# pablojara/kubernetesNetAwareScheduler

Measured on AMD Instinct MI355X. Metric: pod-node pair scores/sec and placements/sec at 10k nodes x 100k pods, higher is better.
Workload: dtype i8xi8->i32; 1 GPU; C3: 10000 nodes x 100000 pods, dense i8 latency + traffic, racks of 32 / zones of 16 racks, 8 peers per pod, clusterloader2-shaped requests; nodes=10000, pods=100000, parallelism=node-sharded x1, candidates_per_pod=8

## Files before the change

kubernetesnetawarescheduler_amd/csrc/k_cost.hip:

```cpp
#include "klist.h"

#include <type_traits>

namespace nas {
namespace {

typedef int v4i __attribute__((ext_vector_type(4)));
typedef int v16i __attribute__((ext_vector_type(16)));
typedef float v16f __attribute__((ext_vector_type(16)));
typedef float v4f __attribute__((ext_vector_type(4)));
typedef __bf16 bf16x8 __attribute__((ext_vector_type(8)));

constexpr int BM = COST_BM;
constexpr int BN = COST_BN;
constexpr int BKB = COST_BKB;
constexpr int PG_NARROW = 4;
constexpr int PG_WIDE = 2;
constexpr int WIDE_PODS = 384;
template <int DT>
constexpr bool mfma16() { return DT == NAS_DT_BF16; }
template <int DT>
struct Mma;

template <>
struct Mma<NAS_DT_I8> {
    using acc_t = v16i;
    using acc4_t = v4i;
    static __device__ __forceinline__ acc_t mma(v4i a, v4i b, acc_t c) {
        return __builtin_amdgcn_mfma_i32_32x32x32_i8(a, b, c, 0, 0, 0);
    }
    static __device__ __forceinline__ acc4_t mma16(v4i a, v4i b, acc4_t c) {
        return __builtin_amdgcn_mfma_i32_16x16x64_i8(a, b, c, 0, 0, 0);
    }
    static __device__ __forceinline__ unsigned okey(int x) { return (unsigned)x ^ 0x80000000u; }
};

template <>
struct Mma<NAS_DT_BF16> {
    using acc_t = v16f;
    using acc4_t = v4f;
    static __device__ __forceinline__ acc_t mma(v4i a, v4i b, acc_t c) {
        return __builtin_amdgcn_mfma_f32_32x32x16_bf16(__builtin_bit_cast(bf16x8, a),
                                                        __builtin_bit_cast(bf16x8, b), c, 0, 0, 0);
    }
    static __device__ __forceinline__ acc4_t mma16(v4i a, v4i b, acc4_t c) {
        return __builtin_amdgcn_mfma_f32_16x16x32_bf16(__builtin_bit_cast(bf16x8, a),
                                                        __builtin_bit_cast(bf16x8, b), c, 0, 0, 0);
    }
    static __device__ __forceinline__ unsigned okey(float x) {
        x = x + 0.0f;
        const unsigned u = __float_as_uint(x);
        return (u & 0x80000000u) ? ~u : (u | 0x80000000u);
    }
};

__device__ __forceinline__ void glds16(const void *g, void *l) {
    __builtin_amdgcn_global_load_lds((const void __attribute__((address_space(1))) *)g,
                                     (void __attribute__((address_space(3))) *)l, 16, 0, 0);
}

__device__ __forceinline__ unsigned lds_off(const void *p) {
    return (unsigned)(uintptr_t)(const __attribute__((address_space(3))) void *)p;
}
__device__ __forceinline__ void glds16_s(const void *sbase, unsigned voff, unsigned ldsa) {
    unsigned keep;
    asm volatile("s_mov_b32 %0, m0\n\ts_mov_b32 m0, %3\n\ts_nop 0\n\t"
                 "global_load_lds_dwordx4 %1, %2\n\ts_mov_b32 m0, %0"
                 : "=&s"(keep)
                 : "v"(voff), "s"(sbase), "s"(ldsa)
                 : "memory");
}

__device__ __forceinline__ unsigned umed3(unsigned a, unsigned b, unsigned c) {
    unsigned d;
    asm("v_med3_u32 %0, %1, %2, %3" : "=v"(d) : "v"(a), "v"(b), "v"(c));
    return d;
}

template <int DT, bool RMAP, int NWN, bool FUSE>
__global__ void __launch_bounds__(128 * NWN, 1)
k_cost_topk(const unsigned char *__restrict__ Lt, const unsigned char *__restrict__ WA, int Kb,
            int n_mt, int n_nt, int p0, int Pp, const u64 *__restrict__ mask,
            u64 *__restrict__ partial, u64 *__restrict__ pbound, int node_base,
            const int *__restrict__ dyn_start, int dyn_hi, const int *__restrict__ dyn_hi_ptr,
            Ovf ov, const int *__restrict__ rowmap, FitSrc fs, unsigned *__restrict__ cc) {
    static_assert(NWN == 4 || NWN == 6, "the 8- and 12-wave layouts");
    constexpr int NW = 2 * NWN;
    constexpr int NI = 2;
    constexpr int WPODS = 32 * NI;
    constexpr int BNK = NWN * WPODS;
    constexpr bool WIDE = BNK > BN;
    static_assert(!WIDE || (!RMAP && FUSE), "the wide tile serves the main pass only");
    static_assert(!FUSE || !RMAP, "the fused fit: main-range launches");
    constexpr int STG = (BM + BNK) * BKB;
    constexpr int PG = WIDE ? PG_WIDE : PG_NARROW;
    constexpr int PPWA = (BM / 8 + NW - 1) / NW;
    constexpr int PPWB = (BNK / 8 + NW - 1) / NW;
    constexpr int PPW = PPWB;
    using M = Mma<DT>;
    using acc_t = typename M::acc_t;
    constexpr bool M16 = mfma16<DT>();
    constexpr int AM = M16 ? 8 : 4;
    constexpr int AN = M16 ? 2 * NI : NI;
    constexpr int AR = M16 ? 4 : 16;
    constexpr int PB = M16 ? 16 : 32;
    using accb_t = std::conditional_t<M16, typename M::acc4_t, acc_t>;
    extern __shared__ __attribute__((aligned(16))) unsigned char lds[];
    constexpr int FIT_LDS_OFF = 32768;
    static_assert(FIT_LDS_OFF >= NWN * NI * 32 * 9 * 8 &&
                  FIT_LDS_OFF + NW * AN * 2 * 64 * 8 <= 2 * STG, "fused-fit LDS words");

    const int nwg = n_mt * n_nt;
    const int b = blockIdx.x;
    const int xcd = b & 7, q8 = nwg >> 3, r8 = nwg & 7;
    const int v = (xcd < r8 ? xcd * (q8 + 1) : r8 * (q8 + 1) + (xcd - r8) * q8) + (b >> 3);
    const int gsize = PG * n_mt;
    const int g = v / gsize, r = v % gsize;
    const int first_nt = g * PG;
    const int pg = min(n_nt - first_nt, PG);
    const int mt = r / pg;
    const int nt = first_nt + r % pg;
    const int cb = blockIdx.y;
    if constexpr (FUSE) {
        fs.cap += (size_t)cb * 3 * fs.N;
        fs.req += (size_t)cb * 3 * Pp;
    }
    Lt += (size_t)cb * n_mt * BM * Kb;
    WA += (size_t)cb * Pp * Kb;
    mask += (size_t)cb * (n_mt * BM / 64) * Pp;
    partial += (size_t)cb * n_mt * Pp * KC;
    pbound += (size_t)cb * n_mt * Pp;
    if (dyn_start) {
        const int s = dyn_start[cb * STATUS_INTS];
        if (s < 0) return;
        if (dyn_hi_ptr) dyn_hi = dyn_hi_ptr[cb * STATUS_INTS];
        p0 = s / BN * BN;
        if (p0 + nt * BNK >= dyn_hi) return;
    }
    const int p_end = (BNK != BN && !dyn_start) ? dyn_hi : 0x7fffffff;

    const int tid = threadIdx.x;
    int lane = tid & 63;
    const int w = WIDE ? __builtin_amdgcn_readfirstlane(tid >> 6) : tid >> 6;
    const int wm = w / NWN, wn = w % NWN;

    const unsigned char *Ag = Lt + (size_t)mt * BM * Kb;
    const unsigned char *Bg = WA + (size_t)(p0 + nt * BNK) * Kb;

    const int srow_in = lane >> 3;
    const int sq = lane & 7;
    auto abuf = [&](int b) -> unsigned char * { return lds + b * STG; };
    auto bbuf = [&](int b) -> unsigned char * { return lds + b * STG + BM * BKB; };
    const unsigned loffn = (unsigned)(srow_in * Kb) +
                           ((unsigned)(sq ^ ((4 * (w & 1) + (srow_in >> 1)) & 7)) << 4);
    auto pieceA = [&](int buf, int k0, int j) {
        if (BM / 8 % NW && j * NW + w >= BM / 8) return;
        const int r0 = (j * NW + w) * 8;
        const int ru = __builtin_amdgcn_readfirstlane(r0);
        glds16_s(Ag + (size_t)ru * Kb + k0, loffn,
                 __builtin_amdgcn_readfirstlane(lds_off(abuf(buf) + r0 * BKB)));
    };
    int bpod[PPW];
    if constexpr (RMAP) {
#pragma unroll
        for (int j = 0; j < PPW; ++j)
            bpod[j] = rowmap[min(p0 + nt * BNK + (j * NW + w) * 8 + srow_in, dyn_hi - 1)];
    }
    auto pieceB = [&](int buf, int k0, int j) {
        if (BNK / 8 % NW && j * NW + w >= BNK / 8) return;
        const int r0 = (j * NW + w) * 8;
        if constexpr (!RMAP) {
            const int ru = __builtin_amdgcn_readfirstlane(r0);
            glds16_s(Bg + (size_t)ru * Kb + k0, loffn,
                     __builtin_amdgcn_readfirstlane(lds_off(bbuf(buf) + r0 * BKB)));
            return;
        }
        const int row = r0 + srow_in;
        const int c = sq ^ ((row >> 1) & 7);
        const unsigned char *src = RMAP ? WA + (size_t)bpod[j] * Kb : Bg + (size_t)row * Kb;
        glds16(src + k0 + c * 16, bbuf(buf) + r0 * BKB);
    };
    const int wu = __builtin_amdgcn_readfirstlane(w);
    const unsigned loff = (unsigned)(srow_in * Kb) +
                          ((unsigned)(sq ^ ((4 * (wu & 1) + (srow_in >> 1)) & 7)) << 4);
    auto piece6 = [&](int buf, int k0, int j) {
        const int pj = j * NW + wu;
        if (pj >= (BM + BNK) / 8) return;
        const unsigned char *base = pj < BM / 8 ? Ag + (size_t)pj * 8 * Kb
                                                : Bg + (size_t)(pj - BM / 8) * 8 * Kb;
        glds16_s(base + k0, loff, __builtin_amdgcn_readfirstlane(lds_off(lds + buf * STG + pj * 8 * BKB)));
    };
    auto stageA = [&](int buf, int k0) {
        if constexpr (WIDE) {
#pragma unroll
            for (int j = 0; j < ((BM + BNK) / 8 + NW - 1) / NW; ++j) piece6(buf, k0, j);
        } else {
#pragma unroll
            for (int j = 0; j < PPWA; ++j) pieceA(buf, k0, j);
        }
    };
    auto stageB = [&](int buf, int k0) {
        if constexpr (!WIDE) {
#pragma unroll
            for (int j = 0; j < PPW; ++j) pieceB(buf, k0, j);
        }
    };

    int rq[FUSE ? AN : 1][3];
    int fcap[2][3];
    auto fit_issue = [&]() {
#pragma unroll
        for (int ni = 0; ni < AN; ++ni) {
            const int pod = min(p0 + nt * BNK + wn * WPODS + ni * PB + (lane & (PB - 1)), p_end - 1);
#pragma unroll
            for (int r = 0; r < 3; ++r) rq[ni][r] = fs.req[(size_t)r * Pp + pod];
        }
#pragma unroll
        for (int mi2 = 0; mi2 < 2; ++mi2) {
            const int nl = mt * BM + wm * 128 + mi2 * 64 + lane;
#pragma unroll
            for (int r = 0; r < 3; ++r)
                fcap[mi2][r] = nl < fs.nloc ? __hip_atomic_load(const_cast<int *>(fs.cap) + (size_t)r * fs.N + fs.n0 + nl,
                                                                __ATOMIC_RELAXED, __HIP_MEMORY_SCOPE_AGENT)
                                            : -1;
        }
    };
    auto fit_slot = [&](int ni, int mi2) -> u64 * {
        return reinterpret_cast<u64 *>(lds + FIT_LDS_OFF) + ((w * AN + ni) * 2 + mi2) * 64 + lane;
    };
    auto fit_words = [&]() {
#pragma unroll
        for (int mi2 = 0; mi2 < 2; ++mi2) {
            const bool real = mt * BM + wm * 128 + mi2 * 64 + lane < fs.nloc;
            const u64 valid = __builtin_amdgcn_ballot_w64(real);
            int mn[3], mx[3];
#pragma unroll
            for (int r = 0; r < 3; ++r) {
                int a = real ? fcap[mi2][r] : 0x7fffffff, x = real ? fcap[mi2][r] : (int)0x80000000;
#pragma unroll
                for (int o = 32; o; o >>= 1) {
                    a = min(a, __shfl_xor(a, o));
                    x = max(x, __shfl_xor(x, o));
                }
                mn[r] = __builtin_amdgcn_readfirstlane(a);
                mx[r] = __builtin_amdgcn_readfirstlane(x);
            }
#pragma unroll
            for (int ni = 0; ni < AN; ++ni) {
                const int a = rq[ni][0], bq = rq[ni][1], d = rq[ni][2];
                const bool all = a <= mn[0] && bq <= mn[1] && d <= mn[2];
                const bool none = a > mx[0] || bq > mx[1] || d > mx[2];
                u64 word = all ? valid : 0ull;
                u64 rest = __builtin_amdgcn_ballot_w64(!all && !none) & ((1ull << PB) - 1);
                while (rest) {
                    const int i = (int)__builtin_ctzll(rest);
                    rest &= rest - 1;
                    const int ra = __builtin_amdgcn_readlane(a, i), rb = __builtin_amdgcn_readlane(bq, i);
                    const int rd = __builtin_amdgcn_readlane(d, i);
                    const u64 m = __builtin_amdgcn_ballot_w64(ra <= fcap[mi2][0]) &
                                  __builtin_amdgcn_ballot_w64(rb <= fcap[mi2][1]) &
                                  __builtin_amdgcn_ballot_w64(rd <= fcap[mi2][2]);
                    if ((lane & (PB - 1)) == i) word = m;
                }
                *fit_slot(ni, mi2) = word;
            }
        }
    };

    u64 mwp[AN][2];
    auto load_mask = [&]() __attribute__((always_inline)) {
        if constexpr (!FUSE) {
#pragma unroll
            for (int ni = 0; ni < AN; ++ni)
#pragma unroll
                for (int mi2 = 0; mi2 < 2; ++mi2) {
                    const int pod = min(p0 + nt * BNK + wn * WPODS + ni * PB + (lane & (PB - 1)), p_end - 1);
                    const int chunk = (mt * BM + wm * 128 + mi2 * 64) >> 6;
                    mwp[ni][mi2] = mask[(size_t)chunk * Pp + pod];
                }
        }
    };
    accb_t acc[AM][AN];
#pragma unroll
    for (int i = 0; i < AM; ++i)
#pragma unroll
        for (int j = 0; j < AN; ++j) acc[i][j] = accb_t{};
    int fr = lane & (PB - 1), fh = lane / PB;
    constexpr bool OVF_ROUND2 = WIDE || !FUSE;
    if constexpr (OVF_ROUND2 && DT == NAS_DT_I8) {
        if (ov.ptr) {
            const int cnt_lim = ov.row_count ? *ov.row_count : 0x7fffffff;
            const signed char *lr = ov.Lr + (size_t)cb * ov.N * (n_mt * BM) + mt * BM + wm * 128 + 4 * fh;
#pragma unroll
            for (int ni = 0; ni < AN; ++ni) {
                const int r = p0 + nt * BNK + wn * WPODS + ni * PB + fr;
                int beg = 0, end = 0;
                if (r < cnt_lim && r < p_end) {
                    const int pod = (ov.row_pod ? ov.row_pod[r] : r) + cb * Pp;
                    beg = ov.ptr[pod];
                    end = ov.ptr[pod + 1];
                }
#pragma unroll
                for (int mi = 0; mi < AM; ++mi)
                    for (int j = beg; j < end; ++j) {
                        const int e = ov.e[j];
                        const signed char *row = lr + (size_t)ov.m[j] * (n_mt * BM) + mi * (128 / AM);
#pragma unroll
                        for (int g = 0; g < AR / 4; ++g) {
                            const int v = *reinterpret_cast<const int *>(row + 8 * g);
#pragma unroll
                            for (int c = 0; c < 4; ++c)
                                acc[mi][ni][4 * g + c] += e * (int)(signed char)(v >> (8 * c));
                        }
                    }
            }
        }
    }
    auto seed_ovf = [&]() __attribute__((always_inline)) {
        if constexpr (!OVF_ROUND2 && DT == NAS_DT_I8) {
            if (ov.ptr) {
                const int cnt_lim = ov.row_count ? *ov.row_count : 0x7fffffff;
                const signed char *lr = ov.Lr + (size_t)cb * ov.N * (n_mt * BM) + mt * BM + wm * 128 + 4 * fh;
                auto bounds = [&](int ni, int &beg, int &end) {
                    const int r = p0 + nt * BNK + wn * WPODS + ni * PB + fr;
                    beg = end = 0;
                    if (r < cnt_lim && r < p_end) {
                        const int pod = (ov.row_pod ? ov.row_pod[r] : r) + cb * Pp;
                        beg = ov.ptr[pod];
                        end = ov.ptr[pod + 1];
                    }
                };
                {
                    int beg[AN], end[AN];
#pragma unroll
                    for (int ni = 0; ni < AN; ++ni) bounds(ni, beg[ni], end[ni]);
#pragma unroll
                    for (int ni = 0; ni < AN; ++ni)
                        for (int j = beg[ni]; j < end[ni]; ++j) {
                            const int e = ov.e[j];
                            const signed char *row = lr + (size_t)ov.m[j] * (n_mt * BM);
                            int v[AM][AR / 4];
#pragma unroll
                            for (int mi = 0; mi < AM; ++mi)
#pragma unroll
                                for (int g = 0; g < AR / 4; ++g)
                                    v[mi][g] = *reinterpret_cast<const int *>(row + mi * (128 / AM) + 8 * g);
#pragma unroll
                            for (int mi = 0; mi < AM; ++mi)
#pragma unroll
                                for (int g = 0; g < AR / 4; ++g)
#pragma unroll
                                    for (int c = 0; c < 4; ++c)
                                        acc[mi][ni][4 * g + c] += e * (int)(signed char)(v[mi][g] >> (8 * c));
                        }
                }
            }
        }
    };
    if constexpr (WIDE) load_mask();

    auto compute = [&](int buf) {
        const unsigned char *As = abuf(buf);
        const unsigned char *Bs = bbuf(buf);
        if constexpr (M16) {
            const unsigned sw = (unsigned)((fh ^ ((fr >> 1) & 7)) << 4);
            const unsigned ao0 = (unsigned)((wm * 128 + fr) * BKB) + sw;
            const unsigned bo0 = (unsigned)((wn * WPODS + fr) * BKB) + sw;
#pragma unroll
            for (int kk = 0; kk < BKB / 64; ++kk) {
                const unsigned ao = ao0 ^ (unsigned)(kk << 6), bo = bo0 ^ (unsigned)(kk << 6);
                v4i bq[AN];
#pragma unroll
                for (int ni = 0; ni < AN; ++ni)
                    bq[ni] = *reinterpret_cast<const v4i *>(Bs + bo + ni * 16 * BKB);
#pragma unroll
                for (int mi = 0; mi < AM; ++mi) {
                    const v4i aq = *reinterpret_cast<const v4i *>(As + ao + mi * 16 * BKB);
#pragma unroll
                    for (int ni = 0; ni < AN; ++ni) acc[mi][ni] = M::mma16(aq, bq[ni], acc[mi][ni]);
                }
            }
            return;
        } else {
        v4i a[2][4], bb[2][NI];
        auto read = [&](int kk, v4i (&ra)[4], v4i (&rb)[NI]) {
            const unsigned ao = ((unsigned)((wm * 128 + fr) * BKB) + (unsigned)((fh ^ ((fr >> 1) & 7)) << 4)) ^ (unsigned)(kk << 5);
            const unsigned bo = ((unsigned)((wn * WPODS + fr) * BKB) + (unsigned)((fh ^ ((fr >> 1) & 7)) << 4)) ^ (unsigned)(kk << 5);
#pragma unroll
            for (int mi = 0; mi < 4; ++mi)
                ra[mi] = *reinterpret_cast<const v4i *>(As + ao + mi * 32 * BKB);
#pragma unroll
            for (int ni = 0; ni < NI; ++ni)
                rb[ni] = *reinterpret_cast<const v4i *>(Bs + bo + ni * 32 * BKB);
        };
        read(0, a[0], bb[0]);
#pragma unroll
        for (int kk = 0; kk < BKB / 32; ++kk) {
            if (kk + 1 < BKB / 32) read(kk + 1, a[(kk + 1) & 1], bb[(kk + 1) & 1]);
#pragma unroll
            for (int mi = 0; mi < 4; ++mi)
#pragma unroll
                for (int ni = 0; ni < NI; ++ni)
                    acc[mi][ni] = M::mma(a[kk & 1][mi], bb[kk & 1][ni], acc[mi][ni]);
        }
        }
    };

    const int nk = Kb / BKB;
    stageA(0, 0);
    stageB(0, 0);
    seed_ovf();
    if constexpr (!WIDE) load_mask();
    asm volatile("s_waitcnt vmcnt(0)" ::: "memory");
    __syncthreads();
    for (int t = 0; t < nk; ++t) {
        const int cur = t & 1;
        if (t + 1 < nk) {
            stageA(cur ^ 1, (t + 1) * BKB);
            stageB(cur ^ 1, (t + 1) * BKB);
        }
        compute(cur);
        asm volatile("s_waitcnt vmcnt(0)" ::: "memory");
        __syncthreads();
    }

    if constexpr (WIDE) {
        int l;
        asm volatile("v_mbcnt_lo_u32_b32 %0, -1, 0\n\tv_mbcnt_hi_u32_b32 %0, -1, %0" : "=v"(l));
        lane = l;
        fr = l & (PB - 1);
        fh = l / PB;
    }
    if (cc) {
        unsigned *crow = cc + (size_t)cb * Pp * (n_mt * BM) + mt * BM + wm * 128;
#pragma unroll
        for (int ni = 0; ni < AN; ++ni) {
            const int pod = p0 + nt * BNK + wn * WPODS + ni * PB + fr;
            if (pod >= p_end) continue;
            unsigned *d = crow + (size_t)pod * (n_mt * BM);
#pragma unroll
            for (int mi = 0; mi < AM; ++mi)
#pragma unroll
                for (int g = 0; g < AR / 4; ++g) {
                    uint4 v;
                    v.x = M::okey(acc[mi][ni][4 * g + 0]);
                    v.y = M::okey(acc[mi][ni][4 * g + 1]);
                    v.z = M::okey(acc[mi][ni][4 * g + 2]);
                    v.w = M::okey(acc[mi][ni][4 * g + 3]);
                    *reinterpret_cast<uint4 *>(d + (M16 ? mi * 16 + 4 * fh : mi * 32 + 8 * g + 4 * fh)) = v;
                }
        }
    }
    if constexpr (FUSE) {
        fit_issue();
        fit_words();
    }
    auto noff = [&](int mi, int reg) -> int {
        return M16 ? mi * 16 + 4 * fh + reg : mi * 32 + (reg & 3) + 8 * (reg >> 2) + 4 * fh;
    };
    constexpr int XL_OFF = FIT_LDS_OFF + NW * AN * 2 * 64 * 8;
    static_assert(!M16 || XL_OFF + 2 * NWN * WPODS * 9 * 8 <= 2 * STG, "16x16 list image");
    u64 *xl = reinterpret_cast<u64 *>(lds + XL_OFF);
    u64 key[M16 ? 1 : AN][8], bnd[M16 ? 1 : AN];
#pragma unroll
    for (int ni = 0; ni < AN; ++ni) {
        u64 (&kl)[8] = key[M16 ? 0 : ni];
        u64 &bl = bnd[M16 ? 0 : ni];
        u64 mwf[2];
        if constexpr (FUSE) {
#pragma unroll
            for (int mi2 = 0; mi2 < 2; ++mi2) mwf[mi2] = *fit_slot(ni, mi2);
        }
        const u64 *mw = FUSE ? mwf : mwp[ni];
        unsigned u[AM][AR];
        unsigned kmin = 0xffffffffu, kmax = 0u;
        int smin = 0x7fffffff, smax = -0x7fffffff - 1;
#pragma unroll
        for (int mi = 0; mi < AM; ++mi)
#pragma unroll
            for (int reg = 0; reg < AR; ++reg) {
                if constexpr (DT == NAS_DT_I8) {
                    smin = min(smin, (int)acc[mi][ni][reg]);
                    smax = max(smax, (int)acc[mi][ni][reg]);
                } else {
                    u[mi][reg] = M::okey(acc[mi][ni][reg]);
                    kmin = min(kmin, u[mi][reg]);
                    kmax = max(kmax, u[mi][reg]);
                }
            }
        if constexpr (DT == NAS_DT_I8) {
            kmin = M::okey(smin);
            kmax = M::okey(smax);
        }
        auto block_bits = [&](int mi) -> unsigned {
            if constexpr (M16)
                return (unsigned)(mw[mi >> 2] >> ((mi & 3) * 16 + 4 * fh)) & 0xfu;
            else
                return (unsigned)(mw[mi >> 1] >> (32 * (mi & 1)));
        };
        constexpr unsigned ALL_BITS = M16 ? 0xfu : 0xffffffffu;
        auto bitpos = [&](int reg) -> int { return M16 ? reg : (reg & 3) + 8 * (reg >> 2) + 4 * fh; };
        u64 k4[4];
        if (__all(kmax - kmin < (1u << 26) - 1u)) {
            unsigned c0 = 0xffffffffu, c1 = c0, c2 = c0, c3 = c0;
            const bool direct = DT == NAS_DT_I8 && __all(smin >= 0 && smax < (1 << 26) - 1);
            const unsigned kbase = direct ? 0x80000000u : kmin;
            const unsigned nk6 = 0u - ((DT == NAS_DT_I8 ? (unsigned)smin : kmin) << 6);
            auto insert = [&](unsigned x) {
                c3 = umed3(c2, c3, x);
                c2 = umed3(c1, c2, x);
                c1 = umed3(c0, c1, x);
                c0 = min(c0, x);
            };
#pragma unroll
            for (int mi = 0; mi < AM; ++mi) {
                const unsigned bitsw = block_bits(mi);
                const unsigned nbits = ~bitsw;
                if (direct && __all(bitsw == ALL_BITS)) {
#pragma unroll
                    for (int reg = 0; reg < AR; ++reg)
                        insert(((unsigned)(int)acc[mi][ni][reg] << 6) | (unsigned)(mi * AR + reg));
                } else {
#pragma unroll
                    for (int reg = 0; reg < AR; ++reg) {
                        const unsigned raw = DT == NAS_DT_I8 ? (unsigned)(int)acc[mi][ni][reg]
                                                             : u[mi][reg];
                        unsigned y;
                        if (direct) {
                            y = raw << 6;
                        } else {
                            asm("v_lshl_add_u32 %0, %1, 6, %2" : "=v"(y) : "v"(raw), "v"(nk6));
                        }
                        insert(y | (unsigned)(mi * AR + reg) |
                               (unsigned)__builtin_amdgcn_sbfe((int)nbits, bitpos(reg), 1));
                    }
                }
            }
            const unsigned cc[4] = {c0, c1, c2, c3};
            const unsigned nb = (unsigned)(node_base + mt * BM + wm * 128 + 4 * fh);
#pragma unroll
            for (int j = 0; j < 4; ++j) {
                const unsigned i = cc[j] & 63u;
                unsigned node;
                if constexpr (M16) {
                    node = nb + (i >> 2) * 16u + (i & 3u);
                } else {
                    const unsigned r = i & 15u;
                    node = nb + (i >> 4) * 32u + (r & 3u) + 8u * (r >> 2);
                }
                k4[j] = cc[j] == 0xffffffffu ? KEY_INVALID
                                             : ((u64)((cc[j] >> 6) + kbase) << 32) | node;
            }
        } else {
            Top4 t4;
            t4.init();
            const unsigned node0 = (unsigned)(node_base + mt * BM + wm * 128);
#pragma unroll
            for (int mi = 0; mi < AM; ++mi) {
                const unsigned bits = block_bits(mi);
#pragma unroll
                for (int reg = 0; reg < AR; ++reg) {
                    const unsigned key = DT == NAS_DT_I8 ? M::okey(acc[mi][ni][reg]) : u[mi][reg];
                    const unsigned x = key | ((((bits >> bitpos(reg)) & 1u) ^ 1u) * 0xffffffffu);
                    t4.insert(x, node0 + noff(mi, reg));
                }
            }
#pragma unroll
            for (int j = 0; j < 4; ++j) k4[j] = t4.c[j] == 0xffffffffu ? KEY_INVALID : t4.key(j);
        }
        u64 o4[4];
#pragma unroll
        for (int j = 0; j < 4; ++j) o4[j] = shfl_xor64(k4[j], M16 ? 16 : 32);
        merge44(k4, o4, kl);
        bl = umin64(k4[3], o4[3]);
        if constexpr (M16) {
            u64 o8[8];
#pragma unroll
            for (int j = 0; j < 8; ++j) o8[j] = shfl_xor64(kl[j], 32);
            const u64 ob = shfl_xor64(bl, 32);
            merge88(kl, o8);
            bl = umin64(umin64(bl, ob), kl[7]);
            if (fh == (ni & 3)) {
                u64 *d = xl + ((size_t)(wm * NWN + wn) * WPODS + ni * 16 + fr) * 9;
#pragma unroll
                for (int j = 0; j < 8; ++j) d[j] = kl[j];
                d[8] = bl;
            }
        }
    }

    u64 *xk = reinterpret_cast<u64 *>(lds);
    if constexpr (M16) {
        __syncthreads();
        if (wm == 0) {
#pragma unroll
            for (int rr = 0; rr < (WPODS + 63) / 64; ++rr) {
                if (rr * 64 + lane >= WPODS) continue;
                const u64 *d0 = xl + ((size_t)wn * WPODS + rr * 64 + lane) * 9;
                const u64 *d1 = d0 + (size_t)NWN * WPODS * 9;
                u64 mine[8], other[8];
#pragma unroll
                for (int j = 0; j < 8; ++j) {
                    mine[j] = d0[j];
                    other[j] = d1[j];
                }
                merge88(mine, other);
                const u64 bb = umin64(umin64(d0[8], d1[8]), mine[7]);
                const int pod = p0 + nt * BNK + wn * WPODS + rr * 64 + lane;
                if (pod < p_end) {
                    store8(partial + ((size_t)mt * Pp + pod) * KC, mine);
                    pbound[(size_t)mt * Pp + pod] = bb;
                }
            }
        }
        return;
    } else {
    if (wm == 1 && fh == 0) {
#pragma unroll
        for (int ni = 0; ni < NI; ++ni) {
            u64 *d = xk + ((wn * NI + ni) * 32 + fr) * 9;
#pragma unroll
            for (int j = 0; j < 8; ++j) d[j] = key[ni][j];
            d[8] = bnd[ni];
        }
    }
    __syncthreads();
    if (wm == 0) {
        auto finish = [&](u64 (&mine)[8], u64 b, int ni, int rr) {
            u64 other[8];
            const u64 *s = xk + ((wn * NI + ni) * 32 + fr) * 9;
#pragma unroll
            for (int j = 0; j < 8; ++j) other[j] = s[j];
            merge88(mine, other);
            b = umin64(umin64(b, s[8]), mine[7]);
            const int pod = p0 + nt * BNK + wn * WPODS + rr * 64 + lane;
            if (pod >= p_end) return;
            store8(partial + ((size_t)mt * Pp + pod) * KC, mine);
            pbound[(size_t)mt * Pp + pod] = b;
        };
#pragma unroll
        for (int rr = 0; rr < (NI + 1) / 2; ++rr) {
            if (fh == 0) finish(key[2 * rr], bnd[2 * rr], 2 * rr, rr);
            else if (2 * rr + 1 < NI) finish(key[2 * rr + 1], bnd[2 * rr + 1], 2 * rr + 1, rr);
        }
    }
    }
}

constexpr int MERGE_LANES = 8;
constexpr int MERGE_BLOCK = 512;

__global__ void __launch_bounds__(MERGE_BLOCK)
k_merge(const u64 *__restrict__ keys, const u64 *__restrict__ bounds, int n_lists,
        long long stride, long long bstride, int src_p0, int p0, int np,
        u64 *__restrict__ dst, u64 *__restrict__ dst_bound, int dst_p0,
        const int *__restrict__ dyn_start, int dyn_hi, int dyn_flags, long long dst_cs,
        const int *__restrict__ dyn_hi_ptr, const int *__restrict__ dst_idx,
        int *__restrict__ init_status) {
    if (init_status && blockIdx.x == 0 && blockIdx.y == 0 && threadIdx.x < 2 * STATUS_INTS)
        init_status[threadIdx.x] = threadIdx.x == 0 ? -1 : 0;
    const int cb = blockIdx.y;
    keys += (size_t)cb * n_lists * stride;
    bounds += (size_t)cb * n_lists * bstride;
    dst += (size_t)cb * dst_cs * KC;
    dst_bound += (size_t)cb * dst_cs;
    if (dyn_start) {
        const int s = dyn_start[cb * STATUS_INTS];
        if (s < 0) return;
        if (dyn_hi_ptr) dyn_hi = dyn_hi_ptr[cb * STATUS_INTS];
        p0 = s;
        np = min(np, dyn_hi - s);
        if (dyn_flags & MERGE_SRC_WINDOW) src_p0 = s;
        if (dyn_flags & MERGE_DST_WINDOW) dst_p0 = s;
    }
    const int t = blockIdx.x * blockDim.x + threadIdx.x;
    const int i = t / MERGE_LANES, s = t % MERGE_LANES;
    const bool live = i < np;
    const size_t ps = (size_t)(p0 + (live ? i : 0) - src_p0);
    u64 a[8], bb[8];
    u64 bound = KEY_INVALID;
#pragma unroll
    for (int j = 0; j < 8; ++j) a[j] = KEY_INVALID;
    if (live) {
        for (int l = s; l < n_lists; l += MERGE_LANES) {
            load8(keys + l * stride + ps * KC, bb);
            merge88(a, bb);
            bound = umin64(bound, bounds[l * bstride + ps]);
        }
    }
#pragma unroll
    for (int m = 1; m < MERGE_LANES; m <<= 1) {
#pragma unroll
        for (int j = 0; j < 8; ++j) bb[j] = shfl_xor64(a[j], m);
        bound = umin64(bound, shfl_xor64(bound, m));
        merge88(a, bb);
    }
    if (!live || s != 0) return;
    const int r = p0 + i - dst_p0;
    const int p = dst_idx ? dst_idx[r] : r;
    store8(dst + (size_t)p * KC, a);
    dst_bound[p] = umin64(bound, a[7]);
}

template <int DT, bool RMAP, int NWN = 4, bool FUSE = (NWN == 6)>
hipError_t launch_cost_t(hipStream_t st, const void *Lt, const void *WA, int Mp, int Kb, int Pp,
                         int p0, int np, const uint64_t *mask, uint64_t *partial,
                         uint64_t *pbound, int node_base, const Dyn *dyn, int batch,
                         const Ovf &ov, const int32_t *rowmap, const FitSrc &fs = FitSrc{},
                         uint32_t *cache = nullptr) {
    constexpr int BNK = NWN * 64;
    constexpr bool WIDE = BNK > BN;
    const void *fn = reinterpret_cast<const void *>(&k_cost_topk<DT, RMAP, NWN, FUSE>);
    constexpr int lds = 2 * (BM + BNK) * BKB;
    static std::atomic<unsigned long long> attr_set{0};
    hipError_t e = set_lds_once(fn, lds, attr_set);
    if (e != hipSuccess) return e;
    const int n_mt = Mp / BM, n_nt = (np + BNK - 1) / BNK;
    if (WIDE && (int64_t)p0 + (int64_t)n_nt * BNK > (int64_t)Pp + WA_PAD_ROWS)
        return hipErrorInvalidValue;
    if (FUSE && (!fs.cap || !fs.req || fs.nloc > Mp || fs.n0 + fs.nloc > fs.N || dyn))
        return hipErrorInvalidValue;
    auto *lt = static_cast<const unsigned char *>(Lt);
    auto *wa = static_cast<const unsigned char *>(WA);
    auto *mk = reinterpret_cast<const u64 *>(mask);
    auto *pa = reinterpret_cast<u64 *>(partial);
    auto *pb = reinterpret_cast<u64 *>(pbound);
    const int *ds = dyn ? dyn->start : nullptr;
    const int dh = dyn ? dyn->hi : 0;
    const int *dhp = dyn ? dyn->hi_ptr : nullptr;
    const int dhi = WIDE ? p0 + np : dh;
    k_cost_topk<DT, RMAP, NWN, FUSE><<<dim3(n_mt * n_nt, batch), 128 * NWN, lds, st>>>(
        lt, wa, Kb, n_mt, n_nt, p0, Pp, mk, pa, pb, node_base, ds, dhi, dhp, ov, rowmap, fs,
        reinterpret_cast<unsigned *>(cache));
    return hipGetLastError();
}

}

int cost_tile_pods(int) { return WIDE_PODS; }

hipError_t launch_cost_topk(hipStream_t st, int dtype, const void *Lt, const void *WA, int Mp,
                            int Kp, int Pp, int p0, int np, const uint64_t *mask,
                            uint64_t *partial, uint64_t *pbound, int node_base, const Dyn *dyn,
                            int batch, const Ovf *ovf, const int32_t *rowmap, bool wide,
                            const FitSrc *fit, uint32_t *cache) {
    if (fit && (dyn || rowmap)) return hipErrorInvalidValue;
    if (cache && (dyn || rowmap)) return hipErrorInvalidValue;
    if (!fit && wide && !dyn && !rowmap) return hipErrorInvalidValue;
    const Ovf ov = ovf ? *ovf : Ovf{};
    if (rowmap && (!dyn || batch != 1)) return hipErrorInvalidValue;
#define NAS_COST_DISPATCH(DTV, KB, OVV)                                                            \
    (rowmap ? launch_cost_t<DTV, true>(st, Lt, WA, Mp, KB, Pp, p0, np, mask, partial, pbound,     \
                                       node_base, dyn, batch, OVV, rowmap)                        \
     : (!dyn && wide)                                                                             \
            ? launch_cost_t<DTV, false, 6>(st, Lt, WA, Mp, KB, Pp, p0, np, mask, partial, pbound, \
                                           node_base, dyn, batch, OVV, nullptr, *fit, cache)      \
     : fit ? launch_cost_t<DTV, false, 4, true>(st, Lt, WA, Mp, KB, Pp, p0, np,     \
                                                             mask, partial, pbound, node_base,    \
                                                             dyn, batch, OVV, nullptr, *fit,      \
                                                             cache)                               \
            : launch_cost_t<DTV, false>(st, Lt, WA, Mp, KB, Pp, p0, np, mask, partial, pbound,    \
                                        node_base, dyn, batch, OVV, nullptr, FitSrc{}, cache))
    if (dyn) {
        p0 = 0;
        np = (int)round_up(dyn->win, BN) + BN;
        if (!dyn->hi_ptr && dyn->hi > Pp) return hipErrorInvalidValue;
    }
    if (np <= 0) return hipSuccess;
    if (Mp % BM || np % BN || (!dyn && p0 + np > Pp)) return hipErrorInvalidValue;
    if (dtype == NAS_DT_I8) {
        if (Kp % BKB) return hipErrorInvalidValue;
        return NAS_COST_DISPATCH(NAS_DT_I8, Kp, ov);
    }
    if (dtype != NAS_DT_BF16) return hipErrorInvalidValue;
    if ((2 * Kp) % BKB) return hipErrorInvalidValue;
    return NAS_COST_DISPATCH(NAS_DT_BF16, 2 * Kp, Ovf{});
#undef NAS_COST_DISPATCH
}

hipError_t launch_merge(hipStream_t st, const uint64_t *keys, const uint64_t *bounds, int n_lists,
                        int64_t stride, int64_t bstride, int src_p0, int p0, int np,
                        uint64_t *cand_key, uint64_t *cand_bound, int dst_p0, const Dyn *dyn,
                        int dyn_flags, int batch, int64_t dst_cluster_pods,
                        const int32_t *dst_idx, int32_t *init_status) {
    if (dyn) np = dyn->win;
    if (np <= 0) return hipSuccess;
    if (dst_idx && batch != 1) return hipErrorInvalidValue;
    if (init_status && (dyn || batch != 1)) return hipErrorInvalidValue;
    k_merge<<<dim3((int)(((int64_t)np * MERGE_LANES + MERGE_BLOCK - 1) / MERGE_BLOCK), batch),
              MERGE_BLOCK, 0, st>>>(
        reinterpret_cast<const u64 *>(keys), reinterpret_cast<const u64 *>(bounds), n_lists, stride,
        bstride, src_p0, p0, np, reinterpret_cast<u64 *>(cand_key),
        reinterpret_cast<u64 *>(cand_bound), dst_p0, dyn ? dyn->start : nullptr, dyn ? dyn->hi : 0,
        dyn_flags, (long long)dst_cluster_pods, dyn ? dyn->hi_ptr : nullptr, dst_idx, init_status);
    return hipGetLastError();
}

}
```

kubernetesnetawarescheduler_amd/csrc/klist.h:

```cpp
#pragma once

#include "nas_internal.h"

namespace nas {

typedef unsigned long long u64;
static_assert(KC == 8, "list networks are written for 8 candidates");

__device__ __forceinline__ u64 umin64(u64 a, u64 b) { return a < b ? a : b; }
__device__ __forceinline__ u64 umax64(u64 a, u64 b) { return a < b ? b : a; }
__device__ __forceinline__ void cex(u64 &a, u64 &b) {
    const u64 lo = umin64(a, b);
    b = umax64(a, b);
    a = lo;
}

__device__ __forceinline__ void bitonic8(u64 (&x)[8]) {
    cex(x[0], x[4]); cex(x[1], x[5]); cex(x[2], x[6]); cex(x[3], x[7]);
    cex(x[0], x[2]); cex(x[1], x[3]); cex(x[4], x[6]); cex(x[5], x[7]);
    cex(x[0], x[1]); cex(x[2], x[3]); cex(x[4], x[5]); cex(x[6], x[7]);
}

__device__ __forceinline__ void merge44(const u64 (&a)[4], const u64 (&b)[4], u64 (&out)[8]) {
    out[0] = a[0]; out[1] = a[1]; out[2] = a[2]; out[3] = a[3];
    out[4] = b[3]; out[5] = b[2]; out[6] = b[1]; out[7] = b[0];
    bitonic8(out);
}

__device__ __forceinline__ void merge88(u64 (&a)[8], const u64 (&b)[8]) {
#pragma unroll
    for (int i = 0; i < 8; ++i) a[i] = umin64(a[i], b[7 - i]);
    bitonic8(a);
}

__device__ __forceinline__ u64 shfl_xor64(u64 x, int m) {
    const int lo = __shfl_xor((int)(unsigned)x, m);
    const int hi = __shfl_xor((int)(unsigned)(x >> 32), m);
    return ((u64)(unsigned)hi << 32) | (unsigned)lo;
}

struct Top4 {
    unsigned c[4], n[4];
    __device__ __forceinline__ void init() {
#pragma unroll
        for (int j = 0; j < 4; ++j) c[j] = n[j] = 0xffffffffu;
    }
    __device__ __forceinline__ void insert(unsigned x, unsigned node) {
        const bool b0 = x < c[0], b1 = x < c[1], b2 = x < c[2], b3 = x < c[3];
        const unsigned c3 = b2 ? c[2] : (b3 ? x : c[3]), n3 = b2 ? n[2] : (b3 ? node : n[3]);
        const unsigned c2 = b1 ? c[1] : (b2 ? x : c[2]), n2 = b1 ? n[1] : (b2 ? node : n[2]);
        const unsigned c1 = b0 ? c[0] : (b1 ? x : c[1]), n1 = b0 ? n[0] : (b1 ? node : n[1]);
        c[0] = b0 ? x : c[0];
        n[0] = b0 ? node : n[0];
        c[1] = c1; n[1] = n1; c[2] = c2; n[2] = n2; c[3] = c3; n[3] = n3;
    }
    __device__ __forceinline__ u64 key(int j) const { return ((u64)c[j] << 32) | n[j]; }
};

__device__ __forceinline__ void load8(const u64 *p, u64 (&k)[8]) {
    const ulonglong2 *s = reinterpret_cast<const ulonglong2 *>(p);
#pragma unroll
    for (int i = 0; i < 4; ++i) {
        const ulonglong2 v = s[i];
        k[2 * i] = v.x;
        k[2 * i + 1] = v.y;
    }
}

__device__ __forceinline__ void store8(u64 *p, const u64 (&k)[8]) {
    ulonglong2 *d = reinterpret_cast<ulonglong2 *>(p);
#pragma unroll
    for (int i = 0; i < 4; ++i) d[i] = make_ulonglong2(k[2 * i], k[2 * i + 1]);
}

}
```

Measured before the change: 139.1 billion pair-scores/s.

## Pack top-k epilogue keys into 32-bit words when scores fit in 24 bits

The i8 epilogue now checks whether all accumulator values in the wave fit in 24 bits. If so, it packs score and local node index into one 32-bit key and runs the top-4/top-8 insertion and merge networks on 32-bit values. Keys are widened to 64-bit only at the final store. It also replaces the shuffle-based min/max reductions with DPP plus readlane, and uses permlane32_swap to merge the two half-wave lists instead of 64-bit shuffles. The cross-wave LDS exchange now holds one list per lane and a per-wave flag selecting 32- or 64-bit format. This adds branching and code size in exchange for cheaper epilogue sorting and exchange.

```diff
diff --git a/kubernetesnetawarescheduler_amd/csrc/k_cost.hip b/kubernetesnetawarescheduler_amd/csrc/k_cost.hip
--- a/kubernetesnetawarescheduler_amd/csrc/k_cost.hip
+++ b/kubernetesnetawarescheduler_amd/csrc/k_cost.hip
@@ -75,6 +75,17 @@
     unsigned d;
     asm("v_med3_u32 %0, %1, %2, %3" : "=v"(d) : "v"(a), "v"(b), "v"(c));
     return d;
+}
+
+template <bool MAX>
+__device__ __forceinline__ int wave_minmax(int v) {
+    auto op = [](int a, int b) { return MAX ? max(a, b) : min(a, b); };
+    v = op(v, __builtin_amdgcn_mov_dpp(v, 0xB1, 0xf, 0xf, true));
+    v = op(v, __builtin_amdgcn_mov_dpp(v, 0x4E, 0xf, 0xf, true));
+    v = op(v, __builtin_amdgcn_mov_dpp(v, 0x141, 0xf, 0xf, true));
+    v = op(v, __builtin_amdgcn_mov_dpp(v, 0x140, 0xf, 0xf, true));
+    return op(op(__builtin_amdgcn_readlane(v, 0), __builtin_amdgcn_readlane(v, 16)),
+              op(__builtin_amdgcn_readlane(v, 32), __builtin_amdgcn_readlane(v, 48)));
 }
 
 template <int DT, bool RMAP, int NWN, bool FUSE>
@@ -218,11 +229,11 @@
 #pragma unroll
         for (int mi2 = 0; mi2 < 2; ++mi2) {
             const int nl = mt * BM + wm * 128 + mi2 * 64 + lane;
+            const int nc = min(fs.n0 + max(min(nl, fs.nloc - 1), 0), fs.N - 1);
 #pragma unroll
             for (int r = 0; r < 3; ++r)
-                fcap[mi2][r] = nl < fs.nloc ? __hip_atomic_load(const_cast<int *>(fs.cap) + (size_t)r * fs.N + fs.n0 + nl,
-                                                                __ATOMIC_RELAXED, __HIP_MEMORY_SCOPE_AGENT)
-                                            : -1;
+                fcap[mi2][r] = __hip_atomic_load(const_cast<int *>(fs.cap) + (size_t)r * fs.N + nc,
+                                                 __ATOMIC_RELAXED, __HIP_MEMORY_SCOPE_AGENT);
         }
     };
     auto fit_slot = [&](int ni, int mi2) -> u64 * {
@@ -233,17 +244,12 @@
         for (int mi2 = 0; mi2 < 2; ++mi2) {
             const bool real = mt * BM + wm * 128 + mi2 * 64 + lane < fs.nloc;
             const u64 valid = __builtin_amdgcn_ballot_w64(real);
-            int mn[3], mx[3];
+            int mn[3], mx[3], fc[3];
 #pragma unroll
             for (int r = 0; r < 3; ++r) {
-                int a = real ? fcap[mi2][r] : 0x7fffffff, x = real ? fcap[mi2][r] : (int)0x80000000;
-#pragma unroll
-                for (int o = 32; o; o >>= 1) {
-                    a = min(a, __shfl_xor(a, o));
-                    x = max(x, __shfl_xor(x, o));
-                }
-                mn[r] = __builtin_amdgcn_readfirstlane(a);
-                mx[r] = __builtin_amdgcn_readfirstlane(x);
+                mn[r] = wave_minmax<false>(real ? fcap[mi2][r] : 0x7fffffff);
+                mx[r] = wave_minmax<true>(real ? fcap[mi2][r] : (int)0x80000000);
+                fc[r] = real ? fcap[mi2][r] : -1;
             }
 #pragma unroll
             for (int ni = 0; ni < AN; ++ni) {
@@ -257,9 +263,9 @@
                     rest &= rest - 1;
                     const int ra = __builtin_amdgcn_readlane(a, i), rb = __builtin_amdgcn_readlane(bq, i);
                     const int rd = __builtin_amdgcn_readlane(d, i);
-                    const u64 m = __builtin_amdgcn_ballot_w64(ra <= fcap[mi2][0]) &
-                                  __builtin_amdgcn_ballot_w64(rb <= fcap[mi2][1]) &
-                                  __builtin_amdgcn_ballot_w64(rd <= fcap[mi2][2]);
+                    const u64 m = __builtin_amdgcn_ballot_w64(ra <= fc[0]) &
+                                  __builtin_amdgcn_ballot_w64(rb <= fc[1]) &
+                                  __builtin_amdgcn_ballot_w64(rd <= fc[2]);
                     if ((lane & (PB - 1)) == i) word = m;
                 }
                 *fit_slot(ni, mi2) = word;
@@ -431,6 +437,21 @@
         fr = l & (PB - 1);
         fh = l / PB;
     }
+    if constexpr (FUSE && !M16) fit_issue();
+    unsigned umx[M16 ? 1 : AN];
+    if constexpr (!M16) {
+#pragma unroll
+        for (int ni = 0; ni < AN; ++ni) {
+            unsigned hi = 0u;
+#pragma unroll
+            for (int mi = 0; mi < AM; ++mi)
+#pragma unroll
+                for (int reg = 0; reg < AR; ++reg) hi = max(hi, (unsigned)(int)acc[mi][ni][reg]);
+            umx[ni] = hi;
+        }
+    }
+    bool use24 = false;
+    if constexpr (!M16) use24 = __all(max(umx[0], umx[1]) < (1u << 24) - 1u);
     if (cc) {
         unsigned *crow = cc + (size_t)cb * Pp * (n_mt * BM) + mt * BM + wm * 128;
 #pragma unroll
@@ -452,20 +473,29 @@
         }
     }
     if constexpr (FUSE) {
-        fit_issue();
+        if constexpr (M16) fit_issue();
         fit_words();
     }
+    static_assert(M16 == (DT == NAS_DT_BF16) && (M16 || NI == 2), "epilogue layouts");
+    const unsigned tile_node0 = (unsigned)(node_base + mt * BM);
+    auto widen = [&](unsigned x) -> u64 {
+        return x == 0xffffffffu ? KEY_INVALID
+                                : ((u64)((x >> 8) + 0x80000000u) << 32) | (tile_node0 + (x & 255u));
+    };
     auto noff = [&](int mi, int reg) -> int {
         return M16 ? mi * 16 + 4 * fh + reg : mi * 32 + (reg & 3) + 8 * (reg >> 2) + 4 * fh;
     };
     constexpr int XL_OFF = FIT_LDS_OFF + NW * AN * 2 * 64 * 8;
     static_assert(!M16 || XL_OFF + 2 * NWN * WPODS * 9 * 8 <= 2 * STG, "16x16 list image");
     u64 *xl = reinterpret_cast<u64 *>(lds + XL_OFF);
-    u64 key[M16 ? 1 : AN][8], bnd[M16 ? 1 : AN];
+    constexpr int XF_OFF = FIT_LDS_OFF - 64;
+    static_assert(NWN * WPODS * 9 * 8 <= XF_OFF && NWN * 4 <= 64, "cross-wave list image");
+    u64 kl[8], bl = KEY_INVALID;
+    u64 k4s[M16 ? 1 : AN][4];
+    unsigned c24[M16 ? 1 : AN][4];
 #pragma unroll
     for (int ni = 0; ni < AN; ++ni) {
-        u64 (&kl)[8] = key[M16 ? 0 : ni];
-        u64 &bl = bnd[M16 ? 0 : ni];
+        u64 (&k4)[4] = k4s[M16 ? 0 : ni];
         u64 mwf[2];
         if constexpr (FUSE) {
 #pragma unroll
@@ -475,22 +505,24 @@
         unsigned u[AM][AR];
         unsigned kmin = 0xffffffffu, kmax = 0u;
         int smin = 0x7fffffff, smax = -0x7fffffff - 1;
-#pragma unroll
-        for (int mi = 0; mi < AM; ++mi)
-#pragma unroll
-            for (int reg = 0; reg < AR; ++reg) {
-                if constexpr (DT == NAS_DT_I8) {
-                    smin = min(smin, (int)acc[mi][ni][reg]);
-                    smax = max(smax, (int)acc[mi][ni][reg]);
-                } else {
-                    u[mi][reg] = M::okey(acc[mi][ni][reg]);
-                    kmin = min(kmin, u[mi][reg]);
-                    kmax = max(kmax, u[mi][reg]);
-                }
-            }
-        if constexpr (DT == NAS_DT_I8) {
-            kmin = M::okey(smin);
-            kmax = M::okey(smax);
+        if (!use24) {
+#pragma unroll
+            for (int mi = 0; mi < AM; ++mi)
+#pragma unroll
+                for (int reg = 0; reg < AR; ++reg) {
+                    if constexpr (DT == NAS_DT_I8) {
+                        smin = min(smin, (int)acc[mi][ni][reg]);
+                        smax = max(smax, (int)acc[mi][ni][reg]);
+                    } else {
+                        u[mi][reg] = M::okey(acc[mi][ni][reg]);
+                        kmin = min(kmin, u[mi][reg]);
+                        kmax = max(kmax, u[mi][reg]);
+                    }
+                }
+            if constexpr (DT == NAS_DT_I8) {
+                kmin = M::okey(smin);
+                kmax = M::okey(smax);
+            }
         }
         auto block_bits = [&](int mi) -> unsigned {
             if constexpr (M16)
@@ -500,7 +532,40 @@
         };
         constexpr unsigned ALL_BITS = M16 ? 0xfu : 0xffffffffu;
         auto bitpos = [&](int reg) -> int { return M16 ? reg : (reg & 3) + 8 * (reg >> 2) + 4 * fh; };
-        u64 k4[4];
+        if constexpr (!M16) {
+            if (use24) {
+                unsigned c0 = 0xffffffffu, c1 = c0, c2 = c0, c3 = c0;
+                auto insert = [&](unsigned x) {
+                    c3 = umed3(c2, c3, x);
+                    c2 = umed3(c1, c2, x);
+                    c1 = umed3(c0, c1, x);
+                    c0 = min(c0, x);
+                };
+#pragma unroll
+                for (int mi = 0; mi < AM; ++mi) {
+                    const unsigned bitsw = block_bits(mi);
+                    const unsigned nbits = ~bitsw;
+                    if (__all(bitsw == ALL_BITS)) {
+#pragma unroll
+                        for (int reg = 0; reg < AR; ++reg)
+                            insert(((unsigned)(int)acc[mi][ni][reg] << 8) |
+                                   (unsigned)(mi * 32 + 8 * (reg >> 2) + (reg & 3)));
+                    } else {
+#pragma unroll
+                        for (int reg = 0; reg < AR; ++reg)
+                            insert(((unsigned)(int)acc[mi][ni][reg] << 8) |
+                                   (unsigned)(mi * 32 + 8 * (reg >> 2) + (reg & 3)) |
+                                   (unsigned)__builtin_amdgcn_sbfe((int)nbits, bitpos(reg), 1));
+                    }
+                }
+                const unsigned hb = (unsigned)(fh << 2 | wm << 7);
+                c24[ni][0] = c0 | hb;
+                c24[ni][1] = c1 | hb;
+                c24[ni][2] = c2 | hb;
+                c24[ni][3] = c3 | hb;
+                continue;
+            }
+        }
         if (__all(kmax - kmin < (1u << 26) - 1u)) {
             unsigned c0 = 0xffffffffu, c1 = c0, c2 = c0, c3 = c0;
             const bool direct = DT == NAS_DT_I8 && __all(smin >= 0 && smax < (1 << 26) - 1);
@@ -568,12 +633,12 @@
 #pragma unroll
             for (int j = 0; j < 4; ++j) k4[j] = t4.c[j] == 0xffffffffu ? KEY_INVALID : t4.key(j);
         }
-        u64 o4[4];
-#pragma unroll
-        for (int j = 0; j < 4; ++j) o4[j] = shfl_xor64(k4[j], M16 ? 16 : 32);
-        merge44(k4, o4, kl);
-        bl = umin64(k4[3], o4[3]);
         if constexpr (M16) {
+            u64 o4[4];
+#pragma unroll
+            for (int j = 0; j < 4; ++j) o4[j] = shfl_xor64(k4[j], 16);
+            merge44(k4, o4, kl);
+            bl = umin64(k4[3], o4[3]);
             u64 o8[8];
 #pragma unroll
             for (int j = 0; j < 8; ++j) o8[j] = shfl_xor64(kl[j], 32);
@@ -615,35 +680,70 @@
         }
         return;
     } else {
-    if (wm == 1 && fh == 0) {
-#pragma unroll
-        for (int ni = 0; ni < NI; ++ni) {
-            u64 *d = xk + ((wn * NI + ni) * 32 + fr) * 9;
-#pragma unroll
-            for (int j = 0; j < 8; ++j) d[j] = key[ni][j];
-            d[8] = bnd[ni];
-        }
-    }
-    __syncthreads();
-    if (wm == 0) {
-        auto finish = [&](u64 (&mine)[8], u64 b, int ni, int rr) {
-            u64 other[8];
-            const u64 *s = xk + ((wn * NI + ni) * 32 + fr) * 9;
-#pragma unroll
-            for (int j = 0; j < 8; ++j) other[j] = s[j];
-            merge88(mine, other);
-            b = umin64(umin64(b, s[8]), mine[7]);
-            const int pod = p0 + nt * BNK + wn * WPODS + rr * 64 + lane;
+        unsigned kl32[8], bl32 = 0xffffffffu;
+        if (use24) {
+#pragma unroll
+            for (int j = 0; j < 4; ++j) half_swap(c24[0][j], c24[1][j]);
+            merge44(c24[0], c24[1], kl32);
+            bl32 = min(c24[0][3], c24[1][3]);
+        } else {
+#pragma unroll
+            for (int j = 0; j < 4; ++j) half_swap(k4s[0][j], k4s[1][j]);
+            merge44(k4s[0], k4s[1], kl);
+            bl = umin64(k4s[0][3], k4s[1][3]);
+        }
+        unsigned *xk32 = reinterpret_cast<unsigned *>(lds);
+        unsigned *xf = reinterpret_cast<unsigned *>(lds + XF_OFF);
+        const int slot = (wn * WPODS + lane) * 9;
+        const int slot32 = wn * WPODS * 18 + lane * 9;
+        if (wm == 1) {
+            if (use24) {
+#pragma unroll
+                for (int j = 0; j < 8; ++j) xk32[slot32 + j] = kl32[j];
+                xk32[slot32 + 8] = bl32;
+            } else {
+#pragma unroll
+                for (int j = 0; j < 8; ++j) xk[slot + j] = kl[j];
+                xk[slot + 8] = bl;
+            }
+            if (lane == 0) xf[wn] = use24 ? 1u : 0u;
+        }
+        __syncthreads();
+        if (wm == 0) {
+            const bool o24 = __builtin_amdgcn_readfirstlane(xf[wn]) != 0;
+            if (use24 && o24) {
+                unsigned other[8];
+#pragma unroll
+                for (int j = 0; j < 8; ++j) other[j] = xk32[slot32 + j];
+                merge88(kl32, other);
+                bl32 = min(min(bl32, xk32[slot32 + 8]), kl32[7]);
+#pragma unroll
+                for (int j = 0; j < 8; ++j) kl[j] = widen(kl32[j]);
+                bl = widen(bl32);
+            } else {
+                if (use24) {
+#pragma unroll
+                    for (int j = 0; j < 8; ++j) kl[j] = widen(kl32[j]);
+                    bl = widen(bl32);
+                }
+                u64 other[8], ob;
+                if (o24) {
+#pragma unroll
+                    for (int j = 0; j < 8; ++j) other[j] = widen(xk32[slot32 + j]);
+                    ob = widen(xk32[slot32 + 8]);
+                } else {
+#pragma unroll
+                    for (int j = 0; j < 8; ++j) other[j] = xk[slot + j];
+                    ob = xk[slot + 8];
+                }
+                merge88(kl, other);
+                bl = umin64(umin64(bl, ob), kl[7]);
+            }
+            const int pod = p0 + nt * BNK + wn * WPODS + lane;
             if (pod >= p_end) return;
-            store8(partial + ((size_t)mt * Pp + pod) * KC, mine);
-            pbound[(size_t)mt * Pp + pod] = b;
-        };
-#pragma unroll
-        for (int rr = 0; rr < (NI + 1) / 2; ++rr) {
-            if (fh == 0) finish(key[2 * rr], bnd[2 * rr], 2 * rr, rr);
-            else if (2 * rr + 1 < NI) finish(key[2 * rr + 1], bnd[2 * rr + 1], 2 * rr + 1, rr);
-        }
-    }
+            store8(partial + ((size_t)mt * Pp + pod) * KC, kl);
+            pbound[(size_t)mt * Pp + pod] = bl;
+        }
     }
 }
 
diff --git a/kubernetesnetawarescheduler_amd/csrc/klist.h b/kubernetesnetawarescheduler_amd/csrc/klist.h
--- a/kubernetesnetawarescheduler_amd/csrc/klist.h
+++ b/kubernetesnetawarescheduler_amd/csrc/klist.h
@@ -14,23 +14,46 @@
     b = umax64(a, b);
     a = lo;
 }
+__device__ __forceinline__ void cex(unsigned &a, unsigned &b) {
+    const unsigned lo = min(a, b);
+    b = max(a, b);
+    a = lo;
+}
+__device__ __forceinline__ unsigned kmin2(unsigned a, unsigned b) { return min(a, b); }
+__device__ __forceinline__ u64 kmin2(u64 a, u64 b) { return umin64(a, b); }
 
-__device__ __forceinline__ void bitonic8(u64 (&x)[8]) {
+template <typename T>
+__device__ __forceinline__ void bitonic8(T (&x)[8]) {
     cex(x[0], x[4]); cex(x[1], x[5]); cex(x[2], x[6]); cex(x[3], x[7]);
     cex(x[0], x[2]); cex(x[1], x[3]); cex(x[4], x[6]); cex(x[5], x[7]);
     cex(x[0], x[1]); cex(x[2], x[3]); cex(x[4], x[5]); cex(x[6], x[7]);
 }
 
-__device__ __forceinline__ void merge44(const u64 (&a)[4], const u64 (&b)[4], u64 (&out)[8]) {
+template <typename T>
+__device__ __forceinline__ void merge44(const T (&a)[4], const T (&b)[4], T (&out)[8]) {
     out[0] = a[0]; out[1] = a[1]; out[2] = a[2]; out[3] = a[3];
     out[4] = b[3]; out[5] = b[2]; out[6] = b[1]; out[7] = b[0];
     bitonic8(out);
 }
 
-__device__ __forceinline__ void merge88(u64 (&a)[8], const u64 (&b)[8]) {
+template <typename T>
+__device__ __forceinline__ void merge88(T (&a)[8], const T (&b)[8]) {
 #pragma unroll
-    for (int i = 0; i < 8; ++i) a[i] = umin64(a[i], b[7 - i]);
+    for (int i = 0; i < 8; ++i) a[i] = kmin2(a[i], b[7 - i]);
     bitonic8(a);
+}
+
+__device__ __forceinline__ void half_swap(unsigned &a, unsigned &b) {
+    const auto r = __builtin_amdgcn_permlane32_swap(a, b, false, false);
+    a = r[0];
+    b = r[1];
+}
+__device__ __forceinline__ void half_swap(u64 &a, u64 &b) {
+    unsigned al = (unsigned)a, ah = (unsigned)(a >> 32), bl = (unsigned)b, bh = (unsigned)(b >> 32);
+    half_swap(al, bl);
+    half_swap(ah, bh);
+    a = ((u64)ah << 32) | al;
+    b = ((u64)bh << 32) | bl;
 }
 
 __device__ __forceinline__ u64 shfl_xor64(u64 x, int m) {
```

After: 140.2 billion pair-scores/s (median of 6 runs). No clear change (+0.8%).
